# VladimirRadenkovic/Image-inpainting-and-Super-Resolution-using-Diffusion-Models-and-Conditional-Flow-Matching

Hardware: AMD Instinct MI355X
Metric: sampled images/sec (50-step, 32x32) (higher is better)
Workload: dtype bf16

## Files before the change

### image-inpainting-and-super-resolution-using-diffusion-models-and-conditional-flow-matching_amd/csrc/capi.hip

```cpp
#include <cstring>
#include <vector>

#include "capi_internal.h"

static thread_local std::string g_err;
void mi355_set_error(const std::string& msg) { g_err = msg; }

const mi355_debug_config& mi355_default_debug() {
  static const mi355_debug_config d = [] { mi355_debug_config c; mi355_debug_defaults(&c); return c; }();
  return d;
}

extern "C" {

int mi355_version(void) { return 108; }
void mi355_debug_defaults(mi355_debug_config* c) {
  if (!c) return;
  std::memset(c, 0, sizeof(*c));
  c->conv_ws = 3; c->conv_small = 15; c->conv_min_wgs = 512; c->conv_stagger = 0; c->conv_ablate = 0; c->conv_spin_limit = 1 << 22;
  c->conv_time_reps = 0; c->gn_apply_max_hw = 64; c->gn_fuse = 1; c->l2_warm = 1; c->attn_fused = 1; c->gn_epilogue = 7; c->conv_pp = 109; c->conv_edge = 15;
}
int mi355_unet_status(mi355_unet* net, int clear) {
  if (!net) { mi355_set_error("null handle"); return -1; }
  return unet_status(net, clear);
}
const char* mi355_last_error(void) { return g_err.c_str(); }

int mi355_unet_param_count(const mi355_unet_config* cfg) {
  if (!cfg) { mi355_set_error("null config"); return -1; }
  std::vector<ParamInfo> p;
  int rc = unet_enumerate_params(*cfg, p);
  return rc ? rc : (int)p.size();
}

int mi355_unet_param_info(const mi355_unet_config* cfg, int index, char* name, int name_cap, int64_t shape[4], int* ndim) {
  if (!cfg || !name || !shape || !ndim) { mi355_set_error("null argument"); return -1; }
  std::vector<ParamInfo> p;
  if (int rc = unet_enumerate_params(*cfg, p)) return rc;
  MI355_REQUIRE(index >= 0 && index < (int)p.size(), -1, "param index out of range");
  MI355_REQUIRE((int)p[index].name.size() + 1 <= name_cap, -1, "name buffer too small");
  std::strcpy(name, p[index].name.c_str());
  *ndim = (int)p[index].shape.size();
  for (int i = 0; i < 4; ++i) shape[i] = i < *ndim ? p[index].shape[i] : 1;
// ... 273 lines not shown
```

### image-inpainting-and-super-resolution-using-diffusion-models-and-conditional-flow-matching_amd/csrc/common.h

```cpp
#pragma once
#include <hip/hip_runtime.h>
#include <stdint.h>
#include <atomic>
#include <cstring>
#include <string>

typedef __bf16 bf16;
typedef _Float16 f16;
typedef float f32x4 __attribute__((ext_vector_type(4)));
typedef float f32x2 __attribute__((ext_vector_type(2)));
typedef __bf16 bf16x8 __attribute__((ext_vector_type(8)));
typedef __bf16 bf16x4 __attribute__((ext_vector_type(4)));
typedef _Float16 f16x8 __attribute__((ext_vector_type(8)));
typedef _Float16 f16x4 __attribute__((ext_vector_type(4)));
typedef _Float16 f16x2 __attribute__((ext_vector_type(2)));
typedef uint32_t u32x4 __attribute__((ext_vector_type(4)));
typedef uint32_t u32x2 __attribute__((ext_vector_type(2)));

template <typename T> struct Elem;
template <> struct Elem<float> {
  static constexpr int CHUNK = 16;
  static constexpr int VEC = 4;
  static constexpr int DTYPE = 0;
};
// ... 106 lines not shown
  const uint64_t bit = 1ull << (dev & 63);
  if (done.load(std::memory_order_acquire) & bit) return 0;
  hipError_t e = hipFuncSetAttribute(reinterpret_cast<const void*>(kern), hipFuncAttributeMaxDynamicSharedMemorySize, 160 * 1024);
  if (e != hipSuccess) {
    (void)hipGetLastError();
    mi355_set_error(std::string(what) + ": hipFuncSetAttribute(MaxDynamicSharedMemorySize, 160 KB) failed: " + hipGetErrorString(e));
    return -3;
  }
  done.fetch_or(bit, std::memory_order_release);
  return 0;
}

__device__ __forceinline__ void l2_warm_wave(const void* p, uint32_t bytes) {
  const uint32_t rank = blockIdx.x >> 3, per = (gridDim.x + 7) >> 3, step = per * 64u * 128u;
  const char* base = reinterpret_cast<const char*>(p);
  uint32_t off = (rank * 64u + (threadIdx.x & 63)) * 128u;
  uint32_t v[16];
#pragma unroll
  for (int i = 0; i < 16; ++i, off += step) v[i] = *reinterpret_cast<const uint32_t*>(base + (off < bytes ? off : 0u));
#pragma unroll
  for (int i = 0; i < 16; ++i) asm volatile("" ::"v"(v[i]));
}

template <int NI>
struct GnPartial {
  f32x2 s2[NI], q2[NI];
  __device__ __forceinline__ GnPartial() {
#pragma unroll
    for (int i = 0; i < NI; ++i) { s2[i] = f32x2{0.f, 0.f}; q2[i] = f32x2{0.f, 0.f}; }
  }
  __device__ __forceinline__ void add(int ni, float v0, float v1, float v2, float v3, bool masked, float valid) {
    f32x2 lo = f32x2{v0, v1}, hi = f32x2{v2, v3};
    if (masked) { lo *= f32x2{valid, valid}; hi *= f32x2{valid, valid}; }
    s2[ni] += lo + hi;
    q2[ni] = lo * lo + q2[ni];
    q2[ni] = hi * hi + q2[ni];
  }
  static __device__ __forceinline__ float row_sum(float v) {
    v += __builtin_bit_cast(float, __builtin_amdgcn_update_dpp(0, __builtin_bit_cast(int, v), 0x140, 0xf, 0xf, false));
    v += __builtin_bit_cast(float, __builtin_amdgcn_update_dpp(0, __builtin_bit_cast(int, v), 0x141, 0xf, 0xf, false));
    v += __builtin_bit_cast(float, __builtin_amdgcn_update_dpp(0, __builtin_bit_cast(int, v), 0x4E, 0xf, 0xf, false));
    v += __builtin_bit_cast(float, __builtin_amdgcn_update_dpp(0, __builtin_bit_cast(int, v), 0xB1, 0xf, 0xf, false));
    return v;
  }
  __device__ __forceinline__ void store(float* dst, int lq, int lr) {
    float ms = 0.f, mq = 0.f;
// ... 9 lines not shown
```

### image-inpainting-and-super-resolution-using-diffusion-models-and-conditional-flow-matching_amd/csrc/conv_igemm.hip

```cpp
#include "conv_kargs.h"

namespace {

template <typename T, int BM, int BN, int WM, int WN, int KS, int PIT, bool MULTI>
__global__ void __launch_bounds__(64 * WM * WN, WM * WN / 2) conv_igemm_kernel(ConvKArgs p) {
  constexpr int NTHREADS = 64 * WM * WN;
  constexpr int FR = NTHREADS / 4;
  using E = Elem<T>;
  constexpr int V = E::VEC, CHUNK = E::CHUNK, ESZ = sizeof(T);
  constexpr bool FAST = (E::DTYPE == 1);
  constexpr int WTM = BM / WM, WTN = BN / WN, MI = WTM / 16, NI = WTN / 16;
  constexpr int WTILE = BN * 64;
  constexpr int WIT = (3 * WTILE + NTHREADS * 16 - 1) / (NTHREADS * 16);
  constexpr int NPL = KS == 1 ? 3 : 1;
  constexpr int WD = (KS == 3 && BM == 64) ? 3 : 1;
  constexpr int PLANE = PIT * FR * PROW;
  static_assert(WM * WN == 4 || WM * WN == 8, "4 or 8 waves");
  extern __shared__ __attribute__((aligned(16))) char smem[];
  char* patch = smem;
  char* wlds = smem + NPL * PLANE;

  const int tid = threadIdx.x, lane = tid & 63, wave = tid >> 6;
  const int wm = wave / WN, wn = wave % WN;
  const int lr = lane & 15, lq = lane >> 4;
// ... 579 lines not shown
}

int conv_launch(const ConvDesc& d, hipStream_t stream) { ConvRoute r; int rc = conv_route(d, &r); return rc ? rc : conv_launch(d, r, stream); }

int conv_launch(const ConvDesc& d, const ConvRoute& r, hipStream_t stream) {
  switch (r.kernel) {
    case CONV_K_1X1_PP: return pp1_launch(d, r, stream);
    case CONV_K_1X1: return conv1x1_launch(d, r, stream);
    case CONV_K_OUT: return conv_out_launch(d, r, stream);
    case CONV_K_IN: return conv_in_launch(d, r, stream);
    default: break;
  }
  ConvPre pre{};
  Geo& g = pre.g;
  ConvKArgs& a = pre.a;
  compute_geo(d, g);
  if (int rc = igemm_args(d, g, a)) return rc;
  pre.K = d.knobs ? d.knobs : &mi355_default_debug();
  if (r.gn_slots) { a.gn_stats = d.gn_stats; a.gn_slots = r.gn_slots; }
  if (r.act_done & 1) {
    a.act_out = d.act_out; a.act_gamma = d.act_gamma; a.act_beta = d.act_beta; a.act_film = d.act_film; a.act_film_stride = d.act_film_stride;
    a.act_eps = d.act_eps; a.act_silu = d.act_silu; a.act_raw = d.act_raw;
  }
  int rc;
  if (r.kernel == CONV_K_PP) rc = pp_launch(d, pre, r, stream);
  else if (r.kernel == CONV_K_WS) rc = ws_launch(d, pre, r, stream);
  else if (r.kernel == CONV_K_SMALL) rc = small_launch(d, pre, r, stream);
  else {
    const dim3 grid(g.groups * g.tiles_x * g.tiles_y, (d.Cout + g.BN - 1) / g.BN);
    rc = dispatch_dtype(d.dtype, [&](auto t) { return launch_cfg<decltype(t)>(a, g.BM, g.BN, d.ks, g.pit_t, grid, g.lds, stream); });
  }
  if (rc) return rc;
  MI355_CHECK_HIP(hipGetLastError());
  return 0;
}
```

### image-inpainting-and-super-resolution-using-diffusion-models-and-conditional-flow-matching_amd/csrc/conv_kargs.h

```cpp
#pragma once
#include "ops.h"

#ifndef WS_ABLATE
#define WS_ABLATE 0
#endif

namespace {

constexpr int PROW = 96;

struct ConvKArgs {
  const void* src0; const void* src1;
  int C0, C1, Cin, nchunks;
  int nreal;
  int N, Hs, Ws, Hc, Wc, Ho, Wo;
  int mode, pad, stride;
  const float* pro_a; const float* pro_b; int pro_silu;
  const void* w; const float* bias; int Cout; int bn_pack;
  const float* emb; int emb_stride;
  const void* res; int res_mode; int Hr, Wr;
  void* out; int out_mode;
  float* gn_stats; int gn_slots;
  int lvw, lth, G, PW, PH, NP, tiles_x, tiles_y;
  uint32_t bytes0, bytes1, wbytes, obytes, rbytes;
  unsigned long long* dbg;
  int ablate;
  int stagger;
  uint32_t* err;
  int spin_limit;
  void* act_out; const float* act_gamma; const float* act_beta; const float* act_film; int act_film_stride; float act_eps;
  int act_silu, act_raw;
  int act_stride, act_coff, act_cpg; uint32_t abytes;
  void* act2_out; const float* act2_gamma; const float* act2_beta; int act2_silu, act2_stride, act2_coff, act2_cpg; uint32_t a2bytes;
  const void* warm; uint32_t warm_bytes;
  const void* sk0; const void* sk1; int SC0, SC1; uint32_t skbytes0, skbytes1;
  uint32_t wstride;
};

#ifdef CONV_STAMPS
__device__ __forceinline__ unsigned long long conv_stamp() {
  unsigned long long t;
  __builtin_amdgcn_sched_barrier(0);
  asm volatile("s_memtime %0\n\ts_waitcnt lgkmcnt(0)" : "=s"(t)::"memory");
  __builtin_amdgcn_sched_barrier(0);
  return t;
}
#define STAMP_DECL unsigned long long st_prev = conv_stamp(), st_acc[8] = {0, 0, 0, 0, 0, 0, 0, 0};
#define STAMP(k) { const unsigned long long st_now = conv_stamp(); st_acc[k] += st_now - st_prev; st_prev = st_now; }
#define STAMP_FLUSH if (p.dbg && (threadIdx.x & 63) == 0) { unsigned long long* q = p.dbg + ((size_t)(blockIdx.y * gridDim.x + blockIdx.x) * (blockDim.x / 64) + (threadIdx.x >> 6)) * 8; for (int k = 0; k < 8; ++k) q[k] = st_acc[k]; }
#define CLK_DECL const unsigned long long ck_t0 = __builtin_amdgcn_s_memtime(), ck_r0 = __builtin_amdgcn_s_memrealtime();
#define CLK_FLUSH if (p.dbg && (threadIdx.x & 63) == 0) { unsigned long long* q = p.dbg - 8192 + ((size_t)blockIdx.x * (blockDim.x / 64) + (threadIdx.x >> 6)) * 2; q[0] = __builtin_amdgcn_s_memtime() - ck_t0; q[1] = __builtin_amdgcn_s_memrealtime() - ck_r0; }
#else
#define STAMP_DECL
#define STAMP(k)
#define STAMP_FLUSH
#define CLK_DECL
#define CLK_FLUSH
#endif

// ... 31 lines not shown
```

### image-inpainting-and-super-resolution-using-diffusion-models-and-conditional-flow-matching_amd/csrc/conv_pp.hip

```cpp
#include "conv_kargs.h"

#ifndef PP_IMPL
#define PP_IMPL "conv_pp.inc.h"
#endif
namespace {
#include PP_IMPL
}

int pp_route(const ConvDesc& d, const ConvPre& p, ConvRoute* r) {
  const Geo& g = p.g;
  const ConvKArgs& a = p.a;
  const int mode = p.K->conv_pp, Ho = g.Ho, Wo = g.Wo, Cout = d.Cout;
  if (!(mode & 3) || d.ks != 3 || g.G != 1 || g.bn_pack != 128 || d.out_mode != OUT_NHWC || g.stride != 1) return 1;
  if (p.has_pro && !d.pro_silu) return 1;
  if (a.nchunks < 2 || (a.nchunks & 1)) return 1;
  const bool up_ok = d.mode == CONV_UP2 && d.w_up2 && !d.wsplit && a.res_mode == RES_NONE;
  if (up_ok && (mode & 64) && !p.has_pro && Cout % 256 == 0 && !(Ho & 1) && !(Wo & 1) && Ho >= 32 && Wo >= 32) {
    const int tiles = ((d.Ws + 15) / 16) * ((d.Hs + 15) / 16);
    if ((mode & 3) >= 2 || 4 * d.N * tiles * (Cout / 256) >= ws_num_cus()) {
      r->kernel = CONV_K_PP; r->form = 2; r->w_up2 = 1;
      r->geom.BM = 256; r->geom.BN = 256; r->geom.lds_bytes = pp::D<0>::lds_bytes(false);
      const int slots = 4 * 2 * tiles;
      if (p.gn_ok && slots <= d.gn_slots_cap) r->gn_slots = slots;
      return 0;
    }
  }
  int cfg = -1;
  if (Cout % 256 == 0 && Wo >= 16 && Ho >= 16) cfg = 0;
  else if (Cout % 128 == 0 && (mode & 8) && Wo >= 32 && Ho >= 16) cfg = 1;
  if (cfg < 0) return 1;
  if (p.has_pro && !(mode & (cfg == 0 ? 4 : 16))) return 1;
  const int vw = cfg == 0 ? 16 : 32, bn = cfg == 0 ? 256 : 128;
  const int tiles = ((Wo + vw - 1) / vw) * ((Ho + 15) / 16);
  if ((mode & 3) < 2 && d.N * tiles * (Cout / bn) < ws_num_cus()) return 1;
  r->kernel = CONV_K_PP; r->form = cfg;
  r->geom.BM = cfg == 0 ? 256 : 512; r->geom.BN = bn;
  r->geom.lds_bytes = cfg == 0 ? pp::D<0>::lds_bytes(p.has_pro) : pp::D<1>::lds_bytes(p.has_pro);
  const bool act = cfg == 0 && Ho == 16 && Wo == 16 && (Cout == 256 || Cout == 512) && a.res_mode == RES_NONE;
  if (act && d.act_out && (p.K->gn_epilogue & 2) && d.act_out == d.out && !d.act_raw) r->act_done = 1;
  const int slots = (cfg == 0 ? 2 : 4) * tiles;
  if (!r->act_done && p.gn_ok && slots <= d.gn_slots_cap) r->gn_slots = slots;
  return 0;
}

int pp_launch(const ConvDesc& d, const ConvPre& p, const ConvRoute& r, hipStream_t stream) {
  ConvKArgs a = p.a;
  if (r.w_up2) {
    MI355_REQUIRE(d.w_up2, -1, "conv: the route asks for the collapsed up-sampling weights (conv_pack_weights_up2) and the description has none");
    a.w = d.w_up2; a.wbytes = (uint32_t)conv_packed_weight_bytes_up2(d.dtype, d.Cout, d.C0 + d.C1);
  }
  return dispatch_dtype(d.dtype, [&](auto t) { return launch_pp<decltype(t)>(a, r.form, stream); });
}
```

### image-inpainting-and-super-resolution-using-diffusion-models-and-conditional-flow-matching_amd/csrc/conv_pp.inc.h

```cpp
#ifndef PP_ABLATE
#define PP_ABLATE 0
#endif
#ifndef PP_TRACE_TAP0
#define PP_TRACE_TAP0 8
#endif
#ifdef CONV_STAMPS
#define PP_TRACE(k) if (tr_on) { const uint32_t ta = (uint32_t)(LDS_END + ((wave8 * 4 + (tr_tap - PP_TRACE_TAP0)) * 5 + (k)) * 4); uint32_t tv = (uint32_t)st_prev; asm volatile("v_mov_b32 %0, %2\n\tv_mov_b32 %1, %3\n\tds_write_b32 %0, %1" : "=&v"(tr_a), "=&v"(tr_v) : "s"(ta), "s"(tv) : "memory"); }
#define PP_TRACE_BYTES 2048
#else
#define PP_TRACE(k)
#define PP_TRACE_BYTES 0
#endif
namespace pp {
constexpr int NRING = 6, AHEAD = 5;
constexpr int ABUF = 512;
template <int CFG> struct G;
template <> struct G<0> {
  static constexpr int VW = 16, TH = 16, BN = 256, WM = 2, WROWS = 8, NWP = 2, NPW = 3;
  static constexpr int row(int mi) { return mi; }
  static constexpr int col(int mi) { (void)mi; return 0; }
};
template <> struct G<1> {
  static constexpr int VW = 32, TH = 16, BN = 128, WM = 4, WROWS = 4, NWP = 1, NPW = 5;
  static constexpr int row(int mi) { return mi >> 1; }
  static constexpr int col(int mi) { return 16 * (mi & 1); }
};
template <int CFG> struct D : G<CFG> {
  using G<CFG>::VW; using G<CFG>::TH; using G<CFG>::BN; using G<CFG>::NPW;
  static constexpr int PW = VW + 2, PH = TH + 2, NPX = PW * PH, NPIECE = 8 * NPW, PLANE = NPIECE * 1024, AROWB = PW * 64;
  static constexpr int WTAP = BN * 64;
  static constexpr int OFF_PLANE = NRING * WTAP, OFF_AB = OFF_PLANE + 2 * PLANE;
  static constexpr int XBUF = 1024;
  static constexpr size_t lds_bytes(int pro, int act = 0) { return (size_t)OFF_AB + (pro ? 8 * ABUF : 0) + (act ? XBUF : 0); }
  static_assert(NPX <= NPIECE * 16, "plane too small");
};
template <int CFG, int PRO, int TAPS = 9> struct S {
  static constexpr int NWP = G<CFG>::NWP, NPW = G<CFG>::NPW, NAB = PRO ? 2 : 0;
  static_assert(TAPS == 9 || (TAPS == 4 && CFG == 0 && PRO == 0), "the four-tap schedule exists for the wide prologue-free form");
  static constexpr int iss(int i) { return TAPS == 4 ? i >> 1 : (PRO ? 0 : (CFG == 0 ? 2 * i : i)); }
  static constexpr int trn(int i) { return CFG == 0 ? 3 + 2 * i : 3 + i; }
  static constexpr int piece_of(int s) { for (int i = 0; i < NPW; ++i) if (trn(i) == s) return i; return -1; }
  static constexpr int npatch(int s) { int n = 0; for (int i = 0; i < NPW; ++i) n += iss(i) == s ? 1 : 0; return n; }
  static constexpr int ops_of(int s) { return (s == 0 ? NAB : 0) + npatch(s) + NWP; }
  static constexpr int yw(int s) { int n = 0; for (int u = s - 3; u <= s; ++u) n += ops_of(u < 0 ? u + TAPS : u); return n; }
  static constexpr int yp(int s) {
    if (TAPS == 4) {
      if (s != TAPS - 1) return 99;
      int n = NWP;
      for (int v = iss(NPW - 1) + 1; v <= s; ++v) n += ops_of(v);
      return n;
    }
    if (!PRO || piece_of(s + 1) < 0) return 99;
    int n = (NPW - 1 - piece_of(s + 1)) + NWP;
    for (int v = 1; v <= s; ++v) n += ops_of(v);
    return n;
  }
// ... 41 lines not shown
#pragma unroll
  for (int j = 0; j < 2 * NV; ++j) e[j] = -1.4426950408889634f * v[j];
#pragma unroll
  for (int j = 0; j < 2 * NV; ++j) e[j] = __builtin_amdgcn_exp2f(e[j]);
#pragma unroll
  for (int j = 0; j < 2 * NV; ++j) e[j] = 1.0f + e[j];
#pragma unroll
  for (int j = 0; j < 2 * NV; ++j) e[j] = __builtin_amdgcn_rcpf(e[j]);
#pragma unroll
  for (int j = 0; j < 2 * NV; ++j) v[j] = v[j] * e[j];
#pragma unroll
  for (int i = 0; i < NV; ++i) out[i] = pack2(v[2 * i], v[2 * i + 1], T());
}
template <int NV>
__device__ __forceinline__ void pp_pro_words(const uint32_t (&raw)[NV], const float* a, const float* b, uint32_t (&out)[NV], float) {
#pragma unroll
  for (int j = 0; j < NV; ++j) { const float v = a[j] * __builtin_bit_cast(float, raw[j]) + b[j]; out[j] = __builtin_bit_cast(uint32_t, v / (1.0f + expf(-v))); }
}

template <typename T, int CFG, int PRO, int ACT = 0, int UP = 0>
__global__ void __launch_bounds__(512, 2) conv3x3_pp_kernel(ConvKArgs p, int n_mt, int n_nt) {
  constexpr int TAPS = UP ? 4 : 9, KW = UP ? 2 : 3;
  static_assert(UP == 0 || (CFG == 0 && PRO == 0 && ACT == 0), "the phase form is the wide prologue-free kernel");
  using Dg = pp::D<CFG>;
  using Sc = pp::S<CFG, PRO, TAPS>;
  using E = Elem<T>;
  constexpr int NRING = pp::NRING, AHEAD = pp::AHEAD;
  constexpr int VW = Dg::VW, TH = Dg::TH, PW = Dg::PW, NPX = Dg::NPX, PLANE = Dg::PLANE, AROWB = Dg::AROWB, BN = Dg::BN, WTAP = Dg::WTAP;
  constexpr int OFF_PLANE = Dg::OFF_PLANE, OFF_AB = Dg::OFF_AB, NPW = Dg::NPW, NWP = Dg::NWP, WMN = Dg::WM, WROWS = Dg::WROWS;
  constexpr int CHUNK = E::CHUNK, ESZ = sizeof(T);
  constexpr int LDS_END = (int)Dg::lds_bytes(PRO, ACT), OFF_X = (int)Dg::lds_bytes(PRO);
  static_assert(ACT == 0 || CFG == 0, "the fused output GroupNorm needs whole images per tile: wide form at 16 x 16");
  (void)LDS_END; (void)NPX; (void)OFF_AB; (void)OFF_X;
  extern __shared__ __attribute__((aligned(16))) char smem[];

  const int lane = threadIdx.x & 63;
  const int wave8 = __builtin_amdgcn_readfirstlane(threadIdx.x >> 6);
  const int grp = wave8 >> 2;
  const int wm = CFG == 0 ? grp : wave8 >> 1, wn = CFG == 0 ? wave8 & 3 : wave8 & 1;
  const int lr = lane & 15, lq = lane >> 4;
  const int tpi = p.tiles_x * p.tiles_y;
  const int T9 = p.nchunks * TAPS;
  const int npt = p.N * tpi;
  const int ntp = ((n_mt + 7) / 8) * 8 * n_nt;
  auto decode = [&](int t, int& mt, int& nt) {
    const int per = 8 * n_nt, blk = t / per, r = t - blk * per;
    nt = r >> 3; mt = blk * 8 + (r & 7);
  };
  auto next_valid = [&](int t) {
    for (t += gridDim.x; t < ntp; t += gridDim.x) { int mt, nt; decode(t, mt, nt); if (mt < n_mt) break; }
    return t;
  };
  auto origin = [&](int mt, int& n0, int& y0, int& x0, int& ph) {
    ph = UP ? mt / npt : 0;
    if constexpr (UP != 0) mt -= ph * npt;
    const int ng = mt / tpi, rem = mt - ng * tpi;
// ... 135 lines not shown
  auto cinit_load = [&](int t) {
    int mt, nt, n0, y0, x0, ph;
    decode(t, mt, nt);
    origin(mt, n0, y0, x0, ph);
#pragma unroll
    for (int ni = 0; ni < NI; ++ni) {
      const int co = nt * BN + wn * 64 + ni * 16 + 4 * lq;
      f32x4 v = f32x4{0.f, 0.f, 0.f, 0.f};
      if (p.bias) v = *reinterpret_cast<const f32x4*>(p.bias + co);
      if (p.emb) { const f32x4 e = *reinterpret_cast<const f32x4*>(p.emb + (size_t)n0 * p.emb_stride + co); v = f32x4{v[0] + e[0], v[1] + e[1], v[2] + e[2], v[3] + e[3]}; }
      cin[ni] = v;
    }
  };
  auto acc_init = [&]() {
#pragma unroll
    for (int mi = 0; mi < 8; ++mi)
#pragma unroll
      for (int ni = 0; ni < NI; ++ni) acc[mi][ni] = cin[ni];
  };

  constexpr int abl = PP_ABLATE;
  STAMP_DECL
  CLK_DECL
  cinit_load(t_first);
  issue_ab(0);
  issue_patch(IC<0>(), IC<0>(), 0); issue_patch(IC<1>(), IC<0>(), 0); issue_patch(IC<2>(), IC<0>(), 0);
  if constexpr (NPW > 3) issue_patch(IC<3>(), IC<0>(), 0);
  if constexpr (NPW > 4) issue_patch(IC<4>(), IC<0>(), 0);
  if constexpr (NPW > 5) issue_patch(IC<5>(), IC<0>(), 0);
  issue_w(IC<0>()); issue_w(IC<1>()); issue_w(IC<2>()); issue_w(IC<3>()); issue_w(IC<4>());
  acc_init();
  pp_wait_vm<Sc::fill_left()>();
  if constexpr (PRO != 0) {
    transform_piece(IC<0>(), IC<0>()); transform_piece(IC<1>(), IC<0>()); transform_piece(IC<2>(), IC<0>());
    if constexpr (NPW > 3) transform_piece(IC<3>(), IC<0>());
    if constexpr (NPW > 4) transform_piece(IC<4>(), IC<0>());
    if constexpr (NPW > 5) transform_piece(IC<5>(), IC<0>());
    asm volatile("s_waitcnt lgkmcnt(0)" ::: "memory");
  }
  pp_barrier();

  constexpr int EPI_STORES = 8 * NP2;
  const int extra0 = PAIR ? EPI_STORES * (p.res_mode != RES_NONE ? 2 : 1) : 0;
  int extra = 0;

  for (int t = t_first; t < ntp;) {
// ... 158 lines not shown
                unpack2(xa[q], ra[2 * q], ra[2 * q + 1], T());
                unpack2(xb[q], rb[2 * q], rb[2 * q + 1], T());
              }
            }
            float va[4], vb[4];
#pragma unroll
            for (int q = 0; q < 4; ++q) {
              va[q] = HAS_RES ? acc[mi][2 * k][q] + ra[q] : acc[mi][2 * k][q];
              vb[q] = HAS_RES ? acc[mi][2 * k + 1][q] + rb[q] : acc[mi][2 * k + 1][q];
            }
            if constexpr (GNM != 0) {
              gp.add(2 * k, va[0], va[1], va[2], va[3], GNM == 2, vm[j]);
              gp.add(2 * k + 1, vb[0], vb[1], vb[2], vb[3], GNM == 2, vm[j]);
            }
            const u32x2 pa2 = pack4(va, T()), pb2 = pack4(vb, T());
            const auto w0 = __builtin_amdgcn_permlane16_swap(pa2[0], pb2[0], false, false);
            const auto w1 = __builtin_amdgcn_permlane16_swap(pa2[1], pb2[1], false, false);
            __builtin_amdgcn_raw_buffer_store_b128(u32x4{w0[0], w1[0], w0[1], w1[1]}, rso, ovo[j] + k * PSTEP * ESZ, 0, 0);
          }
        }
      }
    };
    auto epi = [&](auto resc, auto gnc) { epi_half(IC<0>(), resc, gnc); epi_half(IC<1>(), resc, gnc); };
    if constexpr (ACT != 0) {
      constexpr bool FASTA = E::DTYPE == 1;
      const int cpg = p.Cout >> 5;
      float gs[NI], gq[NI];
#pragma unroll
      for (int ni = 0; ni < NI; ++ni) {
        float s1 = 0.f, s2 = 0.f;
#pragma unroll
        for (int mi = 0; mi < 8; ++mi)
#pragma unroll
          for (int r4 = 0; r4 < 4; ++r4) { s1 += acc[mi][ni][r4]; s2 += acc[mi][ni][r4] * acc[mi][ni][r4]; }
        gs[ni] = GnPartial<1>::row_sum(s1); gq[ni] = GnPartial<1>::row_sum(s2);
      }
      char* xb = smem + OFF_X;
      if (lr == 0) {
#pragma unroll
        for (int ni = 0; ni < NI; ++ni) *reinterpret_cast<f32x2*>(xb + (wn * 2 + wm) * 128 + (ni * 4 + lq) * 8) = f32x2{gs[ni], gq[ni]};
      }
      asm volatile("s_waitcnt lgkmcnt(0)" ::: "memory");
      pp_barrier();
#pragma unroll
      for (int ni = 0; ni < NI; ++ni) {
        const f32x2 h0 = *reinterpret_cast<const f32x2*>(xb + (wn * 2 + 0) * 128 + (ni * 4 + lq) * 8);
        const f32x2 h1 = *reinterpret_cast<const f32x2*>(xb + (wn * 2 + 1) * 128 + (ni * 4 + lq) * 8);
// ... 36 lines not shown
#pragma unroll
          for (int ni = 0; ni < NI; ++ni) {
            f32x4 o;
#pragma unroll
            for (int j = 0; j < 4; ++j) o[j] = actv(ga[ni][j] * acc[mi][ni][j] + gb[ni][j]);
            __builtin_amdgcn_raw_buffer_store_b128(__builtin_bit_cast(u32x4, o), rso, ovo + ni * 16 * ESZ, 0, 0);
          }
        } else {
#pragma unroll
          for (int k = 0; k < NP2; ++k) {
            float va[4], vb[4];
#pragma unroll
            for (int q = 0; q < 4; ++q) {
              va[q] = actv(ga[2 * k][q] * acc[mi][2 * k][q] + gb[2 * k][q]);
              vb[q] = actv(ga[2 * k + 1][q] * acc[mi][2 * k + 1][q] + gb[2 * k + 1][q]);
            }
            const u32x2 pa2 = pack4(va, T()), pb2 = pack4(vb, T());
            const auto w0 = __builtin_amdgcn_permlane16_swap(pa2[0], pb2[0], false, false);
            const auto w1 = __builtin_amdgcn_permlane16_swap(pa2[1], pb2[1], false, false);
            __builtin_amdgcn_raw_buffer_store_b128(u32x4{w0[0], w1[0], w0[1], w1[1]}, rso, ovo + k * PSTEP * ESZ, 0, 0);
          }
        }
      }
    } else if (p.res_mode != RES_NONE) {
      if (!do_gn) epi(IC<1>(), IC<0>()); else if (!gn_mask) epi(IC<1>(), IC<1>()); else epi(IC<1>(), IC<2>());
    } else {
      if (!do_gn) epi(IC<0>(), IC<0>()); else if (!gn_mask) epi(IC<0>(), IC<1>()); else epi(IC<0>(), IC<2>());
    }
    if (do_gn && ACT == 0) {
      const int rem = UP ? mt - ph * npt - n0 * tpi + ph * tpi : mt - n0 * tpi;
      gp.store(p.gn_stats + (((size_t)n0 * p.gn_slots + rem * WMN + wm) * (size_t)(p.Cout >> 2) + ((nt * BN + wn * 64) >> 2)) * 2, lq, lr);
    }
    acc_init();
    if constexpr (!PAIR) pp_wait_vm<0>();
    else if (p.ablate & 64) pp_wait_vm<0>();
    extra = (!PAIR || (p.ablate & 64)) ? 0 : extra0;
    STAMP(5)
    pp_barrier();
    STAMP(6)
    t = t_next;
  }
  pp_wait_vm<0>();
  STAMP_FLUSH
  CLK_FLUSH
#ifdef CONV_STAMPS
  if (p.dbg && blockIdx.x == 0 && lane < 20) p.dbg[2048 * 8 + wave8 * 20 + lane] = *reinterpret_cast<volatile uint32_t*>(smem + LDS_END + (wave8 * 20 + lane) * 4);
#endif
}

template <typename T, int CFG, int PRO, int ACT = 0, int UP = 0>
int launch_pp_k(ConvKArgs a, hipStream_t s) {
  using Dg = pp::D<CFG>;
  a.lvw = CFG == 0 ? 4 : 5; a.lth = 4; a.PW = Dg::PW; a.PH = Dg::PH; a.NP = Dg::NPX;
  const int Ht = UP ? a.Hs : a.Ho, Wt = UP ? a.Ws : a.Wo;
  a.tiles_x = (Wt + Dg::VW - 1) / Dg::VW; a.tiles_y = (Ht + Dg::TH - 1) / Dg::TH;
  const int n_mt = (UP ? 4 : 1) * a.N * a.tiles_x * a.tiles_y, n_nt = a.Cout / Dg::BN;
  if (int rc = mi355_allow_big_lds(conv3x3_pp_kernel<T, CFG, PRO, ACT, UP>, "conv3x3 (ping-pong)")) return rc;
  const int ntp = ((n_mt + 7) / 8) * 8 * n_nt, ncu = ws_num_cus();
  const int grid = ntp < ncu ? ntp : ncu;
  hipLaunchKernelGGL((conv3x3_pp_kernel<T, CFG, PRO, ACT, UP>), dim3(grid), dim3(512), Dg::lds_bytes(PRO, ACT) + PP_TRACE_BYTES, s, a, n_mt, n_nt);
  return 0;
}

template <typename T>
int launch_pp(const ConvKArgs& a, int cfg, hipStream_t s) {
  if (cfg == 2) return launch_pp_k<T, 0, 0, 0, 1>(a, s);
  if (a.act_out) return a.pro_a ? launch_pp_k<T, 0, 2, 1>(a, s) : launch_pp_k<T, 0, 0, 1>(a, s);
  if (a.pro_a) return cfg == 0 ? launch_pp_k<T, 0, 2>(a, s) : launch_pp_k<T, 1, 2>(a, s);
  return cfg == 0 ? launch_pp_k<T, 0, 0>(a, s) : launch_pp_k<T, 1, 0>(a, s);
}
```

### image-inpainting-and-super-resolution-using-diffusion-models-and-conditional-flow-matching_amd/csrc/ops.h

```cpp
#pragma once
#include "common.h"
#include "../../include/mi355_sampler.h"

const mi355_debug_config& mi355_default_debug();

enum { DT_F32 = 0, DT_BF16 = 1, DT_F16 = 2 };
template <typename F> auto dispatch_dtype(int dtype, F&& f) {
  if (dtype == DT_F32) return f(float());
  if (dtype == DT_F16) return f(f16());
  return f(bf16());
}

enum ConvMode { CONV_UNIT = 0, CONV_STRIDE2 = 1, CONV_UP2 = 2, CONV_POOL2 = 3 };
enum ResMode { RES_NONE = 0, RES_SAME = 1, RES_UP2 = 2, RES_POOL2 = 3 };
enum OutMode { OUT_NHWC = 0, OUT_NCHW_F32 = 1 };

struct ConvDesc {
  int dtype;
  const void* src0 = nullptr; int C0 = 0;
  const void* src1 = nullptr; int C1 = 0;
  int N = 0, Hs = 0, Ws = 0;
  int mode = CONV_UNIT;
  int ks = 3;
  const float* pro_a = nullptr;
  const float* pro_b = nullptr;
  int pro_silu = 0;
  const void* w = nullptr;
  const void* w_up2 = nullptr;
  const float* bias = nullptr;
  int Cout = 0;
  const float* emb = nullptr; int emb_stride = 0;
  const void* res = nullptr; int res_mode = RES_NONE;
  void* out = nullptr; int out_mode = OUT_NHWC;
  float* gn_stats = nullptr; int gn_slots_cap = 0;
  void* dbg = nullptr;
  const mi355_debug_config* knobs = nullptr;
  uint32_t* err = nullptr;
  void* act_out = nullptr; const float* act_gamma = nullptr; const float* act_beta = nullptr;
  const float* act_film = nullptr; int act_film_stride = 0; float act_eps = 1e-5f; int act_silu = 0, act_raw = 1;
  int act_stride = 0, act_coff = 0, act_cpg = 0;
  void* act2_out = nullptr; const float* act2_gamma = nullptr; const float* act2_beta = nullptr;
  int act2_silu = 0, act2_stride = 0, act2_coff = 0, act2_cpg = 0;
  const void* warm = nullptr; uint32_t warm_bytes = 0;
  const void* skip_src0 = nullptr; const void* skip_src1 = nullptr; int skip_C0 = 0, skip_C1 = 0;
  const float* nchw0 = nullptr; const float* nchw1 = nullptr; int nchw_c0 = 0, nchw_c1 = 0;
  float* axpy_x = nullptr; float axpy_scale = 0.f;
  int cin_real = 0;
  int wsplit = 0;
};

struct ConvGeom {
  int Ho, Wo, BM, BN;
  size_t lds_bytes;
  int grid_m, grid_n;
};
enum ConvKernel { CONV_K_IGEMM = 0, CONV_K_1X1, CONV_K_1X1_PP, CONV_K_IN, CONV_K_OUT, CONV_K_PP, CONV_K_WS, CONV_K_SMALL };
struct ConvRoute {
  int kernel = CONV_K_IGEMM;
  ConvGeom geom{};
  int form = 0;
  int BM = 0, GC = 0, ntn = 0;
  int lvw = 0, lth = 0, G = 0, tiles_x = 0, tiles_y = 0;
  int n_mt = 0, n_nt = 0;
  int ksplit = 0, sm[10] = {};
  size_t lds = 0;
  int gn_slots = 0;
  int act_done = 0;
  int axpy = 0, skip = 0;
  int reads_nchw = 0;
  int w_up2 = 0;
};
int conv_route(const ConvDesc& d, ConvRoute* r);
int conv_launch(const ConvDesc& d, const ConvRoute& r, hipStream_t stream);
int conv_launch(const ConvDesc& d, hipStream_t stream);
ConvGeom conv_geometry(const ConvDesc& d);
size_t conv_packed_weight_bytes(int dtype, int Cout, int Cin, int ks, int split = 0);
int conv_tile_n(int Cout);
void conv_pack_weights(int dtype, const float* w_host, int Cout, int Cin, int ks, void* dst_host, int split = 0);
size_t conv_packed_weight_bytes_up2(int dtype, int Cout, int Cin);
void conv_pack_weights_up2(int dtype, const float* w_host, int Cout, int Cin, void* dst_host);
size_t conv_packed_weight_bytes_skip(int dtype, int Cout, int Cin, int Cskip);
void conv_pack_weights_skip(int dtype, const float* w3, const float* w1, int Cout, int Cin, int Cskip, void* dst_host);
int pp1_route(const ConvDesc& d, ConvRoute* r);
int pp1_launch(const ConvDesc& d, const ConvRoute& r, hipStream_t stream);
int conv1x1_route(const ConvDesc& d, ConvRoute* r);
int conv1x1_launch(const ConvDesc& d, const ConvRoute& r, hipStream_t stream);
int conv_in_route(const ConvDesc& d, ConvRoute* r);
int conv_in_launch(const ConvDesc& d, const ConvRoute& r, hipStream_t stream);
int conv_out_route(const ConvDesc& d, ConvRoute* r);
int conv_out_launch(const ConvDesc& d, const ConvRoute& r, hipStream_t stream);
// ... 183 lines not shown
```

### image-inpainting-and-super-resolution-using-diffusion-models-and-conditional-flow-matching_amd/csrc/unet_engine.hip

```cpp
#include "unet_engine.h"

#include <algorithm>
#include <cstring>
#include <map>

namespace {

inline size_t align_up(size_t v, size_t a) { return (v + a - 1) / a * a; }

enum BlockKind { BLK_CONV_IN, BLK_RES, BLK_ATTN, BLK_RESAMPLE_CONV, BLK_RESAMPLE, BLK_OUT };
struct Block {
  std::string prefix;
  int kind, cin, cout;
  int dir = 0;
  bool upsample = false;
  bool push = false, pop = false;
};
std::vector<Block> unet_blocks(const mi355_unet_config& cfg) {
  const int mc = cfg.model_channels, nl = cfg.n_channel_mult;
  auto has_attn = [&](int ds) { for (int i = 0; i < cfg.n_attention_ds; ++i) if (cfg.attention_ds[i] == ds) return true; return false; };
  std::vector<Block> out;
  auto add = [&](const std::string& prefix, int kind, int cin, int cout, int dir = 0) -> Block& {
    Block b; b.prefix = prefix; b.kind = kind; b.cin = cin; b.cout = cout; b.dir = dir;
    out.push_back(b);
// ... 559 lines not shown
  const float* WF(size_t off) const { return reinterpret_cast<const float*>(net->dev_weights + off); }
  int cin(const PlanOp& op) const { return net->tensors[op.src0].C + (op.src1 >= 0 ? net->tensors[op.src1].C : 0); }

  void count_readers() {
    ops.assign(net->ops.size(), OpState());
    tens.assign(net->tensors.size(), TensorState());
    for (size_t j = 0; j < net->ops.size(); ++j) {
      const PlanOp& o = net->ops[j];
      if (o.src0 >= 0) ++tens[o.src0].readers;
      if (o.src1 >= 0) ++tens[o.src1].readers;
      if (o.kind == OP_CONV && o.res >= 0) ++tens[o.res].readers;
      if (apply_site(o)) {
        for (int s : {o.src0, o.src1}) if (s >= 0) tens[s].sites[tens[s].n_sites++] = (int)j;
      }
    }
  }

  void warm_next(size_t oi, const void*& wp, uint32_t& wb, int bit) const {
    if (!(net->knobs.l2_warm & bit) || oi + 1 >= net->ops.size() || net->ops[oi + 1].kind != OP_CONV) return;
    const PlanOp& nx = net->ops[oi + 1];
    wp = net->dev_weights + nx.w_off; wb = (uint32_t)conv_packed_weight_bytes(net->cfg.dtype, nx.Cout, cin(nx), nx.ks, net->wsplit);
  }

  struct ConvSites { size_t act_consumer = 0; int fused[2] = {-1, -1}; };
  void describe_conv(size_t oi, bool skip, ConvDesc& c, ConvSites& r) const {
    const PlanOp& op = net->ops[oi];
    const PlanTensor& s0 = net->tensors[op.src0];
    c.dtype = net->cfg.dtype; c.src0 = v.tensor(op.src0); c.C0 = s0.C; c.src1 = v.tensor(op.src1); c.C1 = op.src1 >= 0 ? net->tensors[op.src1].C : 0;
    c.N = B; c.Hs = s0.H; c.Ws = s0.W; c.mode = op.mode; c.ks = op.ks; c.wsplit = net->wsplit;
    if (op.use_pro && !ops[oi].pro_off) {
      c.pro_a = v.f32(v.l.gna); c.pro_b = v.f32(v.l.gnb); c.pro_silu = op.pro_silu;
      if (op.gn_site >= 0) { const WsView::Site s = v.site(op.gn_site); c.pro_a = s.a; c.pro_b = s.b; }
    }
    c.w = net->dev_weights + op.w_off; c.bias = WF(op.bias_off); c.Cout = op.Cout;
    if (op.has_wu) c.w_up2 = net->dev_weights + op.wu_off;
    if (op.src0 == net->in_tensor) {
      c.cin_real = net->cfg.in_channels;
      if (!net->cfg.differentiable && tens[net->in_tensor].readers == 1) { c.nchw0 = x; c.nchw_c0 = Cx; c.nchw1 = cond; c.nchw_c1 = cond ? Cc : 0; }
    }
    if (op.out_mode == OUT_NCHW_F32 && run.euler_x) { c.axpy_x = run.euler_x; c.axpy_scale = run.euler_dt; }
    if (op.emb_off >= 0) { c.emb = embp + op.emb_off; c.emb_stride = estride; }
    if (op.res >= 0) { c.res = v.tensor(op.res); c.res_mode = op.res_mode; }
    c.out_mode = op.out_mode;
    c.knobs = &net->knobs; c.err = net->err_dev;
    c.out = op.out_mode == OUT_NHWC ? v.tensor(op.dst) : (void*)out;
    if (skip) {
      const PlanOp& sk = net->ops[op.skip_op];
      c.skip_src0 = v.tensor(sk.src0); c.skip_C0 = net->tensors[sk.src0].C;
      c.skip_src1 = v.tensor(sk.src1); c.skip_C1 = sk.src1 >= 0 ? net->tensors[sk.src1].C : 0;
      c.w = net->dev_weights + op.wf_off; c.bias = WF(op.bf_off); c.res = nullptr; c.res_mode = RES_NONE;
    }
    if (op.dst >= 0 && net->tensors[op.dst].stats_cap) { c.gn_stats = v.stats(op.dst); c.gn_slots_cap = net->tensors[op.dst].stats_cap; }
    if (op.dst >= 0 && op.out_mode == OUT_NHWC && op.res < 0 && oi + 2 < net->ops.size() && tens[op.dst].readers == 2) {
      const PlanOp& g = net->ops[oi + 1];
      if (g.kind == OP_GN && g.fin_ok && g.dst < 0 && g.src0 == op.dst && g.src1 < 0 && g.gn_site < 0) {
        for (size_t j = oi + 2; j < net->ops.size() && j <= oi + 3; ++j) {
          const PlanOp& cn = net->ops[j];
          if (cn.kind == OP_CONV && cn.use_pro && cn.src0 == op.dst && cn.src1 < 0 && cn.gn_site < 0) { r.act_consumer = j; break; }
        }
        if (r.act_consumer) {
          c.act_out = c.out; c.act_raw = 0; c.act_gamma = WF(g.gamma_off); c.act_beta = WF(g.beta_off);
          if (g.film_emb_off >= 0) { c.act_film = embp + g.film_emb_off; c.act_film_stride = estride; }
          c.act_silu = net->ops[r.act_consumer].pro_silu;
        }
      }
    }
    if (!c.act_out && op.dst >= 0 && op.out_mode == OUT_NHWC) {
      for (int k = 0; k < tens[op.dst].n_sites; ++k) {
        const int gi = tens[op.dst].sites[k];
        const PlanOp& g = net->ops[gi];
        const bool cat = g.src1 >= 0;
        const int Cg = cin(g);
        const int coff = g.src0 == op.dst ? 0 : net->tensors[g.src0].C;
        if (cat) {
          const int cpg = Cg / 32;
          if (!(net->knobs.gn_epilogue & 4) || g.film_emb_off >= 0 || g.src0 == g.src1 || Cg % 32 || net->tensors[g.src0].C % cpg || net->tensors[g.src1].C % cpg) continue;
        }
        if (!c.act_out) {
          c.act_out = v.tensor(g.dst); c.act_gamma = WF(g.gamma_off) + coff; c.act_beta = WF(g.beta_off) + coff;
          if (g.film_emb_off >= 0) { c.act_film = embp + g.film_emb_off; c.act_film_stride = estride; }
          c.act_silu = g.pro_silu; c.act_stride = Cg; c.act_coff = coff; c.act_cpg = Cg / 32;
          if (!cat || coff == 0) warm_next((size_t)gi, c.warm, c.warm_bytes, 1);
          r.fused[0] = gi;
        } else if (!c.act2_out && g.film_emb_off < 0) {
          c.act2_out = v.tensor(g.dst); c.act2_gamma = WF(g.gamma_off) + coff; c.act2_beta = WF(g.beta_off) + coff;
          c.act2_silu = g.pro_silu; c.act2_stride = Cg; c.act2_coff = coff; c.act2_cpg = Cg / 32;
          r.fused[1] = gi;
        }
      }
      if (c.act_out) c.act_raw = c.act2_out ? 1 : tens[op.dst].readers > 1;
    }
  }
  void settle_conv(size_t oi, const ConvRoute& rt, const ConvSites& r) {
    if (rt.act_done && r.act_consumer) { ops[oi + 1].gn_done = 1; ops[r.act_consumer].pro_off = 1; }
    else if (rt.act_done) {
      for (int k = 0; k < 2; ++k) {
        if (!(rt.act_done & (1 << k)) || r.fused[k] < 0) continue;
        if (++ops[r.fused[k]].site_parts == (net->ops[r.fused[k]].src1 >= 0 ? 2 : 1)) ops[r.fused[k]].gn_done = 1;
      }
    }
    if (net->ops[oi].dst >= 0) tens[net->ops[oi].dst].gn_slots = rt.gn_slots;
  }

  void gn_common(const PlanOp& op, const float*& gamma, const float*& beta, const float*& film, int& film_stride) const {
    gamma = WF(op.gamma_off); beta = WF(op.beta_off);
    if (op.film_emb_off >= 0) { film = embp + op.film_emb_off; film_stride = estride; }
  }
  GnFinDesc describe_gn_finalize(size_t oi) const {
    const PlanOp& op = net->ops[oi];
    const PlanTensor& s0 = net->tensors[op.src0];
    GnFinDesc g; g.stats0 = v.stats(op.src0); g.slots0 = tens[op.src0].gn_slots; g.C0 = s0.C;
    if (op.src1 >= 0) { g.stats1 = v.stats(op.src1); g.slots1 = tens[op.src1].gn_slots; g.C1 = net->tensors[op.src1].C; }
    g.N = B; g.HW = s0.H * s0.W;
    gn_common(op, g.gamma, g.beta, g.film, g.film_stride);
    g.a = v.f32(v.l.gna); g.b = v.f32(v.l.gnb);
    g.dtype = net->cfg.dtype; g.src0 = v.tensor(op.src0); g.src1 = v.tensor(op.src1);
    warm_next(oi, g.warm, g.warm_bytes, 2);
    return g;
  }
  GnDesc describe_gn(size_t oi) const {
    const PlanOp& op = net->ops[oi];
    const PlanTensor& s0 = net->tensors[op.src0];
    GnDesc g; g.dtype = net->cfg.dtype; g.src0 = v.tensor(op.src0); g.C0 = s0.C; g.src1 = v.tensor(op.src1); g.C1 = op.src1 >= 0 ? net->tensors[op.src1].C : 0;
// ... 215 lines not shown
```

Baseline: 1453.

## Fuse GroupNorm finalize into 16x16 conv epilogue writing per-channel scale/shift

Adds an ACT==2 variant of the pipelined 3x3 conv kernel that reduces GroupNorm statistics across the tile, computes group mean/rstd, and writes per-channel (a, b) coefficients directly. This removes the separate GN-finalize launch after qualifying 16x16, 256-channel convs. When the fast variance estimate looks numerically ill-conditioned, the kernel does a second pass over the output to recompute centred statistics. The cost is extra LDS, two more barriers and gamma/beta loads inside the conv epilogue. It is enabled by default through a new gn_epilogue bit.

```diff
diff --git a/image-inpainting-and-super-resolution-using-diffusion-models-and-conditional-flow-matching_amd/csrc/capi.hip b/image-inpainting-and-super-resolution-using-diffusion-models-and-conditional-flow-matching_amd/csrc/capi.hip
--- a/image-inpainting-and-super-resolution-using-diffusion-models-and-conditional-flow-matching_amd/csrc/capi.hip
+++ b/image-inpainting-and-super-resolution-using-diffusion-models-and-conditional-flow-matching_amd/csrc/capi.hip
@@ -18,7 +18,7 @@
   if (!c) return;
   std::memset(c, 0, sizeof(*c));
   c->conv_ws = 3; c->conv_small = 15; c->conv_min_wgs = 512; c->conv_stagger = 0; c->conv_ablate = 0; c->conv_spin_limit = 1 << 22;
-  c->conv_time_reps = 0; c->gn_apply_max_hw = 64; c->gn_fuse = 1; c->l2_warm = 1; c->attn_fused = 1; c->gn_epilogue = 7; c->conv_pp = 109; c->conv_edge = 15;
+  c->conv_time_reps = 0; c->gn_apply_max_hw = 64; c->gn_fuse = 1; c->l2_warm = 1; c->attn_fused = 1; c->gn_epilogue = 15; c->conv_pp = 109; c->conv_edge = 15;
 }
 int mi355_unet_status(mi355_unet* net, int clear) {
   if (!net) { mi355_set_error("null handle"); return -1; }
diff --git a/image-inpainting-and-super-resolution-using-diffusion-models-and-conditional-flow-matching_amd/csrc/common.h b/image-inpainting-and-super-resolution-using-diffusion-models-and-conditional-flow-matching_amd/csrc/common.h
--- a/image-inpainting-and-super-resolution-using-diffusion-models-and-conditional-flow-matching_amd/csrc/common.h
+++ b/image-inpainting-and-super-resolution-using-diffusion-models-and-conditional-flow-matching_amd/csrc/common.h
@@ -152,6 +152,24 @@
   for (int i = 0; i < 16; ++i) asm volatile("" ::"v"(v[i]));
 }
 
+__device__ __forceinline__ bool gn_group_stat(float ts, float tq, float inv, float eps, float& mean, float& rstd) {
+  constexpr float RATIO = 2.0f;
+  mean = ts * inv;
+  const float var = fmaxf(tq * inv - mean * mean, 0.f);
+  rstd = 1.0f / sqrtf(var + eps);
+  return !(mean * mean <= RATIO * var);
+}
+__device__ __forceinline__ void gn_group_redo(float dsum, float dsq, float inv, float eps, float& mean, float& rstd) {
+  const float ds = dsum * inv;
+  const float var = fmaxf(dsq * inv - ds * ds, 0.f);
+  mean = mean + ds;
+  rstd = 1.0f / sqrtf(var + eps);
+}
+__device__ __forceinline__ void gn_channel_ab(float mean, float rstd, float gamma, float beta, float& a, float& b) {
+  a = rstd * gamma;
+  b = fmaf(-mean, a, beta);
+}
+
 template <int NI>
 struct GnPartial {
   f32x2 s2[NI], q2[NI];
diff --git a/image-inpainting-and-super-resolution-using-diffusion-models-and-conditional-flow-matching_amd/csrc/conv_igemm.hip b/image-inpainting-and-super-resolution-using-diffusion-models-and-conditional-flow-matching_amd/csrc/conv_igemm.hip
--- a/image-inpainting-and-super-resolution-using-diffusion-models-and-conditional-flow-matching_amd/csrc/conv_igemm.hip
+++ b/image-inpainting-and-super-resolution-using-diffusion-models-and-conditional-flow-matching_amd/csrc/conv_igemm.hip
@@ -625,6 +625,9 @@
     a.act_out = d.act_out; a.act_gamma = d.act_gamma; a.act_beta = d.act_beta; a.act_film = d.act_film; a.act_film_stride = d.act_film_stride;
     a.act_eps = d.act_eps; a.act_silu = d.act_silu; a.act_raw = d.act_raw;
   }
+  if (r.fin_done) {
+    a.fin_a = d.fin_a; a.fin_b = d.fin_b; a.fin_gamma = d.fin_gamma; a.fin_beta = d.fin_beta; a.fin_eps = d.fin_eps; a.fin_groups = d.fin_groups;
+  }
   int rc;
   if (r.kernel == CONV_K_PP) rc = pp_launch(d, pre, r, stream);
   else if (r.kernel == CONV_K_WS) rc = ws_launch(d, pre, r, stream);
diff --git a/image-inpainting-and-super-resolution-using-diffusion-models-and-conditional-flow-matching_amd/csrc/conv_kargs.h b/image-inpainting-and-super-resolution-using-diffusion-models-and-conditional-flow-matching_amd/csrc/conv_kargs.h
--- a/image-inpainting-and-super-resolution-using-diffusion-models-and-conditional-flow-matching_amd/csrc/conv_kargs.h
+++ b/image-inpainting-and-super-resolution-using-diffusion-models-and-conditional-flow-matching_amd/csrc/conv_kargs.h
@@ -35,6 +35,7 @@
   const void* warm; uint32_t warm_bytes;
   const void* sk0; const void* sk1; int SC0, SC1; uint32_t skbytes0, skbytes1;
   uint32_t wstride;
+  float* fin_a; float* fin_b; const float* fin_gamma; const float* fin_beta; float fin_eps; int fin_groups;
 };
 
 #ifdef CONV_STAMPS
diff --git a/image-inpainting-and-super-resolution-using-diffusion-models-and-conditional-flow-matching_amd/csrc/conv_pp.hip b/image-inpainting-and-super-resolution-using-diffusion-models-and-conditional-flow-matching_amd/csrc/conv_pp.hip
--- a/image-inpainting-and-super-resolution-using-diffusion-models-and-conditional-flow-matching_amd/csrc/conv_pp.hip
+++ b/image-inpainting-and-super-resolution-using-diffusion-models-and-conditional-flow-matching_amd/csrc/conv_pp.hip
@@ -40,6 +40,9 @@
   if (act && d.act_out && (p.K->gn_epilogue & 2) && d.act_out == d.out && !d.act_raw) r->act_done = 1;
   const int slots = (cfg == 0 ? 2 : 4) * tiles;
   if (!r->act_done && p.gn_ok && slots <= d.gn_slots_cap) r->gn_slots = slots;
+  if (d.fin_a && d.fin_b && d.fin_gamma && d.fin_beta && (p.K->gn_epilogue & 8) && cfg == 0 && !p.has_pro && !r->act_done && r->gn_slots == 2 && Ho == 16 && Wo == 16 &&
+      Cout == 256 && (d.fin_groups == 32 || d.fin_groups == 16) && (a.res_mode == RES_NONE || a.res_mode == RES_SAME))
+    r->fin_done = 1;
   return 0;
 }
 
diff --git a/image-inpainting-and-super-resolution-using-diffusion-models-and-conditional-flow-matching_amd/csrc/conv_pp.inc.h b/image-inpainting-and-super-resolution-using-diffusion-models-and-conditional-flow-matching_amd/csrc/conv_pp.inc.h
--- a/image-inpainting-and-super-resolution-using-diffusion-models-and-conditional-flow-matching_amd/csrc/conv_pp.inc.h
+++ b/image-inpainting-and-super-resolution-using-diffusion-models-and-conditional-flow-matching_amd/csrc/conv_pp.inc.h
@@ -31,7 +31,8 @@
   static constexpr int WTAP = BN * 64;
   static constexpr int OFF_PLANE = NRING * WTAP, OFF_AB = OFF_PLANE + 2 * PLANE;
   static constexpr int XBUF = 1024;
-  static constexpr size_t lds_bytes(int pro, int act = 0) { return (size_t)OFF_AB + (pro ? 8 * ABUF : 0) + (act ? XBUF : 0); }
+  static constexpr int FINB = 512;
+  static constexpr size_t lds_bytes(int pro, int act = 0) { return (size_t)OFF_AB + (pro ? 8 * ABUF : 0) + (act == 2 ? 2 * XBUF + 8 * FINB : act ? XBUF : 0); }
   static_assert(NPX <= NPIECE * 16, "plane too small");
 };
 template <int CFG, int PRO, int TAPS = 9> struct S {
@@ -119,6 +120,7 @@
 __global__ void __launch_bounds__(512, 2) conv3x3_pp_kernel(ConvKArgs p, int n_mt, int n_nt) {
   constexpr int TAPS = UP ? 4 : 9, KW = UP ? 2 : 3;
   static_assert(UP == 0 || (CFG == 0 && PRO == 0 && ACT == 0), "the phase form is the wide prologue-free kernel");
+  static_assert(ACT != 2 || PRO == 0, "the finalizing form is prologue-free: the (a, b) rows it writes may be the ones a prologue would read");
   using Dg = pp::D<CFG>;
   using Sc = pp::S<CFG, PRO, TAPS>;
   using E = Elem<T>;
@@ -126,9 +128,9 @@
   constexpr int VW = Dg::VW, TH = Dg::TH, PW = Dg::PW, NPX = Dg::NPX, PLANE = Dg::PLANE, AROWB = Dg::AROWB, BN = Dg::BN, WTAP = Dg::WTAP;
   constexpr int OFF_PLANE = Dg::OFF_PLANE, OFF_AB = Dg::OFF_AB, NPW = Dg::NPW, NWP = Dg::NWP, WMN = Dg::WM, WROWS = Dg::WROWS;
   constexpr int CHUNK = E::CHUNK, ESZ = sizeof(T);
-  constexpr int LDS_END = (int)Dg::lds_bytes(PRO, ACT), OFF_X = (int)Dg::lds_bytes(PRO);
+  constexpr int LDS_END = (int)Dg::lds_bytes(PRO, ACT), OFF_X = (int)Dg::lds_bytes(PRO), OFF_FIN = OFF_X + 2 * Dg::XBUF;
   static_assert(ACT == 0 || CFG == 0, "the fused output GroupNorm needs whole images per tile: wide form at 16 x 16");
-  (void)LDS_END; (void)NPX; (void)OFF_AB; (void)OFF_X;
+  (void)LDS_END; (void)NPX; (void)OFF_AB; (void)OFF_X; (void)OFF_FIN;
   extern __shared__ __attribute__((aligned(16))) char smem[];
 
   const int lane = threadIdx.x & 63;
@@ -310,6 +312,13 @@
   constexpr int abl = PP_ABLATE;
   STAMP_DECL
   CLK_DECL
+  if constexpr (ACT == 2) {
+    const __amdgpu_buffer_rsrc_t rsg = __builtin_amdgcn_make_buffer_rsrc(const_cast<float*>(p.fin_gamma), 0, (uint32_t)p.Cout * 4u, 0x00020000);
+    const __amdgpu_buffer_rsrc_t rsbt = __builtin_amdgcn_make_buffer_rsrc(const_cast<float*>(p.fin_beta), 0, (uint32_t)p.Cout * 4u, 0x00020000);
+    char* dst = smem + OFF_FIN + wave8 * Dg::FINB;
+    __builtin_amdgcn_raw_ptr_buffer_load_lds(rsg, (__attribute__((address_space(3))) void*)dst, 4, (uint32_t)lane * 4u, (uint32_t)(wn * 64) * 4u, 0, 0);
+    __builtin_amdgcn_raw_ptr_buffer_load_lds(rsbt, (__attribute__((address_space(3))) void*)(dst + 256), 4, (uint32_t)lane * 4u, (uint32_t)(wn * 64) * 4u, 0, 0);
+  }
   cinit_load(t_first);
   issue_ab(0);
   issue_patch(IC<0>(), IC<0>(), 0); issue_patch(IC<1>(), IC<0>(), 0); issue_patch(IC<2>(), IC<0>(), 0);
@@ -514,7 +523,7 @@
       }
     };
     auto epi = [&](auto resc, auto gnc) { epi_half(IC<0>(), resc, gnc); epi_half(IC<1>(), resc, gnc); };
-    if constexpr (ACT != 0) {
+    if constexpr (ACT == 1) {
       constexpr bool FASTA = E::DTYPE == 1;
       const int cpg = p.Cout >> 5;
       float gs[NI], gq[NI];
@@ -597,14 +606,99 @@
           }
         }
       }
+    } else if constexpr (ACT == 2) {
+      if (p.res_mode != RES_NONE) epi(IC<1>(), IC<1>()); else epi(IC<0>(), IC<1>());
     } else if (p.res_mode != RES_NONE) {
       if (!do_gn) epi(IC<1>(), IC<0>()); else if (!gn_mask) epi(IC<1>(), IC<1>()); else epi(IC<1>(), IC<2>());
     } else {
       if (!do_gn) epi(IC<0>(), IC<0>()); else if (!gn_mask) epi(IC<0>(), IC<1>()); else epi(IC<0>(), IC<2>());
     }
-    if (do_gn && ACT == 0) {
+    if (do_gn && ACT != 1) {
       const int rem = UP ? mt - ph * npt - n0 * tpi + ph * tpi : mt - n0 * tpi;
       gp.store(p.gn_stats + (((size_t)n0 * p.gn_slots + rem * WMN + wm) * (size_t)(p.Cout >> 2) + ((nt * BN + wn * 64) >> 2)) * 2, lq, lr);
+    }
+    if constexpr (ACT == 2) {
+      const int cpg = p.Cout / p.fin_groups;
+      char* xb = smem + OFF_X;
+      float gs[NI], gq[NI];
+#pragma unroll
+      for (int ni = 0; ni < NI; ++ni) {
+        gs[ni] = GnPartial<1>::row_sum(gp.s2[ni][0] + gp.s2[ni][1]); gq[ni] = GnPartial<1>::row_sum(gp.q2[ni][0] + gp.q2[ni][1]);
+      }
+      if (lr == 0) {
+#pragma unroll
+        for (int ni = 0; ni < NI; ++ni) *reinterpret_cast<f32x2*>(xb + (wn * 2 + wm) * 128 + (ni * 4 + lq) * 8) = f32x2{gs[ni], gq[ni]};
+      }
+      asm volatile("s_waitcnt lgkmcnt(0)" ::: "memory");
+      pp_barrier();
+      const float inv_cnt = 1.0f / ((float)cpg * (float)(p.Ho * p.Wo));
+      float gmean[NI], grstd[NI];
+      bool ill[NI], any_ill = false;
+#pragma unroll
+      for (int ni = 0; ni < NI; ++ni) {
+        const f32x2 h0 = *reinterpret_cast<const f32x2*>(xb + (wn * 2 + 0) * 128 + (ni * 4 + lq) * 8);
+        const f32x2 h1 = *reinterpret_cast<const f32x2*>(xb + (wn * 2 + 1) * 128 + (ni * 4 + lq) * 8);
+        float ts = h0[0] + h1[0], tq = h0[1] + h1[1];
+        ts += __shfl_xor(ts, 16); tq += __shfl_xor(tq, 16);
+        if (cpg >= 16) { ts += __shfl_xor(ts, 32); tq += __shfl_xor(tq, 32); }
+        ill[ni] = gn_group_stat(ts, tq, inv_cnt, p.fin_eps, gmean[ni], grstd[ni]);
+        any_ill = any_ill || ill[ni];
+      }
+      float d1[NI], d2[NI];
+#pragma unroll
+      for (int ni = 0; ni < NI; ++ni) { d1[ni] = 0.f; d2[ni] = 0.f; }
+      if (__any(any_ill)) {
+        pp_wait_vm<0>();
+#pragma unroll
+        for (int mi = 0; mi < 8; ++mi) {
+          const int y = y0 + wm * WROWS + Dg::row(mi), x = x0 + Dg::col(mi) + lr;
+          const uint32_t opix = (uint32_t)((n0 * p.Ho + y) * p.Wo + x);
+#pragma unroll
+          for (int ni = 0; ni < NI; ++ni) {
+            const uint32_t vo = (opix * (uint32_t)p.Cout + (uint32_t)(co_w + ni * 16)) * ESZ;
+            float v4[4];
+            if constexpr (PAIR) {
+              const u32x2 w2 = __builtin_bit_cast(u32x2, __builtin_amdgcn_raw_buffer_load_b64(rso, vo, 0, 17));
+              unpack2(w2[0], v4[0], v4[1], T()); unpack2(w2[1], v4[2], v4[3], T());
+            } else {
+              const f32x4 w4 = __builtin_bit_cast(f32x4, __builtin_amdgcn_raw_buffer_load_b128(rso, vo, 0, 17));
+              v4[0] = w4[0]; v4[1] = w4[1]; v4[2] = w4[2]; v4[3] = w4[3];
+            }
+#pragma unroll
+            for (int r4 = 0; r4 < 4; ++r4) { const float dv = v4[r4] - gmean[ni]; d1[ni] += dv; d2[ni] += dv * dv; }
+          }
+        }
+#pragma unroll
+        for (int ni = 0; ni < NI; ++ni) { d1[ni] = GnPartial<1>::row_sum(d1[ni]); d2[ni] = GnPartial<1>::row_sum(d2[ni]); }
+      }
+      char* xd = xb + Dg::XBUF;
+      if (lr == 0) {
+#pragma unroll
+        for (int ni = 0; ni < NI; ++ni) *reinterpret_cast<f32x2*>(xd + (wn * 2 + wm) * 128 + (ni * 4 + lq) * 8) = f32x2{d1[ni], d2[ni]};
+      }
+      asm volatile("s_waitcnt lgkmcnt(0)" ::: "memory");
+      pp_barrier();
+      float fmean = 0.f, frstd = 0.f;
+#pragma unroll
+      for (int ni = 0; ni < NI; ++ni) {
+        const f32x2 h0 = *reinterpret_cast<const f32x2*>(xd + (wn * 2 + 0) * 128 + (ni * 4 + lq) * 8);
+        const f32x2 h1 = *reinterpret_cast<const f32x2*>(xd + (wn * 2 + 1) * 128 + (ni * 4 + lq) * 8);
+        float ts = h0[0] + h1[0], tq = h0[1] + h1[1];
+        ts += __shfl_xor(ts, 16); tq += __shfl_xor(tq, 16);
+        if (cpg >= 16) { ts += __shfl_xor(ts, 32); tq += __shfl_xor(tq, 32); }
+        if (ill[ni]) gn_group_redo(ts, tq, inv_cnt, p.fin_eps, gmean[ni], grstd[ni]);
+        if (lr == ni) { fmean = gmean[ni]; frstd = grstd[ni]; }
+      }
+      if (wm == 0 && lr < NI) {
+        const char* fb = smem + OFF_FIN + wave8 * Dg::FINB + (lr * 16 + 4 * lq) * 4;
+        const f32x4 fin_g = *reinterpret_cast<const f32x4*>(fb), fin_bt = *reinterpret_cast<const f32x4*>(fb + 256);
+        f32x4 av, bv;
+#pragma unroll
+        for (int j = 0; j < 4; ++j) { float a1, b1; gn_channel_ab(fmean, frstd, fin_g[j], fin_bt[j], a1, b1); av[j] = a1; bv[j] = b1; }
+        const size_t co = (size_t)n0 * p.Cout + nt * BN + wn * 64 + lr * 16 + 4 * lq;
+        *reinterpret_cast<f32x4*>(p.fin_a + co) = av;
+        *reinterpret_cast<f32x4*>(p.fin_b + co) = bv;
+      }
     }
     acc_init();
     if constexpr (!PAIR) pp_wait_vm<0>();
@@ -640,6 +734,7 @@
 template <typename T>
 int launch_pp(const ConvKArgs& a, int cfg, hipStream_t s) {
   if (cfg == 2) return launch_pp_k<T, 0, 0, 0, 1>(a, s);
+  if (a.fin_a) return launch_pp_k<T, 0, 0, 2>(a, s);
   if (a.act_out) return a.pro_a ? launch_pp_k<T, 0, 2, 1>(a, s) : launch_pp_k<T, 0, 0, 1>(a, s);
   if (a.pro_a) return cfg == 0 ? launch_pp_k<T, 0, 2>(a, s) : launch_pp_k<T, 1, 2>(a, s);
   return cfg == 0 ? launch_pp_k<T, 0, 0>(a, s) : launch_pp_k<T, 1, 0>(a, s);
diff --git a/image-inpainting-and-super-resolution-using-diffusion-models-and-conditional-flow-matching_amd/csrc/ops.h b/image-inpainting-and-super-resolution-using-diffusion-models-and-conditional-flow-matching_amd/csrc/ops.h
--- a/image-inpainting-and-super-resolution-using-diffusion-models-and-conditional-flow-matching_amd/csrc/ops.h
+++ b/image-inpainting-and-super-resolution-using-diffusion-models-and-conditional-flow-matching_amd/csrc/ops.h
@@ -42,6 +42,7 @@
   void* act2_out = nullptr; const float* act2_gamma = nullptr; const float* act2_beta = nullptr;
   int act2_silu = 0, act2_stride = 0, act2_coff = 0, act2_cpg = 0;
   const void* warm = nullptr; uint32_t warm_bytes = 0;
+  float* fin_a = nullptr; float* fin_b = nullptr; const float* fin_gamma = nullptr; const float* fin_beta = nullptr; float fin_eps = 1e-5f; int fin_groups = 32;
   const void* skip_src0 = nullptr; const void* skip_src1 = nullptr; int skip_C0 = 0, skip_C1 = 0;
   const float* nchw0 = nullptr; const float* nchw1 = nullptr; int nchw_c0 = 0, nchw_c1 = 0;
   float* axpy_x = nullptr; float axpy_scale = 0.f;
@@ -66,6 +67,7 @@
   size_t lds = 0;
   int gn_slots = 0;
   int act_done = 0;
+  int fin_done = 0;
   int axpy = 0, skip = 0;
   int reads_nchw = 0;
   int w_up2 = 0;
diff --git a/image-inpainting-and-super-resolution-using-diffusion-models-and-conditional-flow-matching_amd/csrc/unet_engine.hip b/image-inpainting-and-super-resolution-using-diffusion-models-and-conditional-flow-matching_amd/csrc/unet_engine.hip
--- a/image-inpainting-and-super-resolution-using-diffusion-models-and-conditional-flow-matching_amd/csrc/unet_engine.hip
+++ b/image-inpainting-and-super-resolution-using-diffusion-models-and-conditional-flow-matching_amd/csrc/unet_engine.hip
@@ -605,7 +605,7 @@
     wp = net->dev_weights + nx.w_off; wb = (uint32_t)conv_packed_weight_bytes(net->cfg.dtype, nx.Cout, cin(nx), nx.ks, net->wsplit);
   }
 
-  struct ConvSites { size_t act_consumer = 0; int fused[2] = {-1, -1}; };
+  struct ConvSites { size_t act_consumer = 0; int fused[2] = {-1, -1}; size_t fin_site = 0; };
   void describe_conv(size_t oi, bool skip, ConvDesc& c, ConvSites& r) const {
     const PlanOp& op = net->ops[oi];
     const PlanTensor& s0 = net->tensors[op.src0];
@@ -646,6 +646,13 @@
           if (g.film_emb_off >= 0) { c.act_film = embp + g.film_emb_off; c.act_film_stride = estride; }
           c.act_silu = net->ops[r.act_consumer].pro_silu;
         }
+      }
+    }
+    if (c.gn_stats && op.out_mode == OUT_NHWC && oi + 1 < net->ops.size()) {
+      const PlanOp& g = net->ops[oi + 1];
+      if (g.kind == OP_GN && g.fin_ok && g.dst < 0 && g.src0 == op.dst && g.src1 < 0 && g.gn_site < 0 && g.film_emb_off < 0) {
+        c.fin_a = v.f32(v.l.gna); c.fin_b = v.f32(v.l.gnb); c.fin_gamma = WF(g.gamma_off); c.fin_beta = WF(g.beta_off);
+        r.fin_site = oi + 1;
       }
     }
     if (!c.act_out && op.dst >= 0 && op.out_mode == OUT_NHWC) {
@@ -682,6 +689,7 @@
         if (++ops[r.fused[k]].site_parts == (net->ops[r.fused[k]].src1 >= 0 ? 2 : 1)) ops[r.fused[k]].gn_done = 1;
       }
     }
+    if (rt.fin_done && r.fin_site) ops[r.fin_site].gn_done = 1;
     if (net->ops[oi].dst >= 0) tens[net->ops[oi].dst].gn_slots = rt.gn_slots;
   }
 
```

Result: no change. 1458, median of 6 (+0.3%).
